# thowell/CALIPSO.jl

Hardware: AMD Instinct MI355X
Metric: Newton steps/sec (n~5k KKT) (higher is better)
Workload: dtype f64; 1 GPU; C3 synthetic dense conic QP: nx=2500 ne=1500 nc=1000 (400 R+ + 200 x SOC3), n=5000 condensed, N=8500 unreduced; ONE system per GPU stepped sequentially (replicas at N > 1); 1 LDL^T factorisation, 6 refinement round(s) per step; refinement_rounds=6

## Files before the change

calipso.jl_amd/__init__.py:

```python
import ctypes as C

import numpy as np

from ._lib import CALLBACK_FN, EVAL_FN, CalipsoHipError, lib

__all__ = ["Solver", "Group", "LDLSolver", "SmallBatch", "Comm", "ordering", "symbolic", "Options", "initialize_b", "solve_b", "CalipsoHipError", "FLAGS", "splitmix_uniform",
           "mfma_f64_peak"]

FLAGS = dict(
    objective=1 << 0, objective_gradient_variables=1 << 1, objective_jacobian_variables_variables=1 << 2,
    equality_constraint=1 << 3, equality_jacobian_variables=1 << 4, equality_dual_jacobian_variables=1 << 5,
    equality_dual_jacobian_variables_variables=1 << 6, cone_constraint=1 << 7, cone_jacobian_variables=1 << 8,
    cone_dual_jacobian_variables=1 << 9, cone_dual_jacobian_variables_variables=1 << 10,
    objective_jacobian_variables_parameters=1 << 11, equality_jacobian_parameters=1 << 12,
    equality_dual_jacobian_variables_parameters=1 << 13, cone_jacobian_parameters=1 << 14,
    cone_dual_jacobian_variables_parameters=1 << 15)
CONE_BARRIER, CONE_BARRIER_GRADIENT, CONE_PRODUCT, CONE_JACOBIAN, CONE_TARGET = 1, 2, 4, 8, 16

STATUS_TEXT = {-1: "inertia correction failure", -2: "cone search failure", -3: "evaluation callback failed",
               -4: "bad argument", -5: "HIP error", -6: "cone layout not supported"}


def _pd(a):
    return a.ctypes.data_as(C.POINTER(C.c_double))
# ... 402 lines not shown
    def newton_steps(self, count, advance=False):
        info = np.zeros(6 * max(int(count), 1))
        status = np.zeros(max(int(count), 1), dtype=np.int32)
        self._check(self._L.calipso_hip_newton_steps(self._h, int(count), int(advance), _pd(info), status.ctypes.data_as(C.POINTER(C.c_int32))), "newton_steps")
        I = info.reshape(-1, 6)
        return [dict(status=int(status[k]), step_size=I[k, 0], step_size_cone_slack_dual=I[k, 1], refinement_rounds=int(I[k, 2]), factorizations=int(I[k, 3]),
                     merit_candidate=I[k, 4], violation_candidate=I[k, 5]) for k in range(int(count))]

    def phase_times(self):
        out = np.zeros(9)
        self._L.calipso_hip_phase_times(self._h, _pd(out))
        return out

    def kernel_times(self):
        out = np.zeros(8)
        self._L.calipso_hip_kernel_times(self._h, _pd(out))
        return out

    def structure_work(self):
        out = np.zeros(8)
        self._check(self._L.calipso_hip_structure_work(self._h, _pd(out)), "structure_work")
        return dict(schur_flops=out[0], packed_doubles=out[1], segment_pairs=int(out[2]), factor_flops=out[3], factor_nnz=out[4], order=int(out[5]), structured=bool(out[6]))

    def padded_nx(self):
        return int(self.kernel_times()[2])

    def device_bytes(self):
        return int(self.kernel_times()[3])

    def analyze_structure(self):
        out = np.zeros(4, dtype=np.int64)
        self._check(self._L.calipso_hip_analyze_structure(self._h, _pi(out)), "analyze_structure")
        return dict(half_bandwidth=int(out[0]), band_blocks=int(out[1]), equality_rows_per_group=int(out[2]), cone_rows_per_group=int(out[3]))

    def clear_structure(self):
        self._check(self._L.calipso_hip_clear_structure(self._h), "clear_structure")

    def set_stage_parallel(self, on=True, batch=1):
        out = np.zeros(4, dtype=np.int64)
        self._check(self._L.calipso_hip_set_stage_parallel(self._h, 1 if on else 0, int(batch), _pi(out)), "set_stage_parallel")
        return dict(levels=int(out[0]), largest_front=int(out[1]), nnz_upper=int(out[2]))

    def set_stage_blocks(self, on=True):
        out = np.zeros(4, dtype=np.int64)
        self._check(self._L.calipso_hip_set_stage_blocks(self._h, 1 if on else 0, _pi(out)), "set_stage_blocks")
        return dict(z_blocks=int(out[0]), hessian_blocks=int(out[1]), segments=int(out[2]), packed_doubles=int(out[3]))
# ... 811 lines not shown
```

calipso.jl_amd/_lib.py:

```python
import ctypes as C
import os

_HERE = os.path.dirname(os.path.abspath(__file__))
LIB_PATH = os.environ.get("CALIPSO_HIP_LIB") or os.path.join(_HERE, "libcalipso_hip.so")
_LIB = None

EVAL_FN = C.CFUNCTYPE(C.c_int32, C.c_void_p, C.c_uint32, C.POINTER(C.c_double), C.POINTER(C.c_double), C.POINTER(C.c_double),
                      C.POINTER(C.c_double))

CALLBACK_FN = C.CFUNCTYPE(None, C.c_void_p, C.c_void_p)
DEVICE_EVAL_FN = C.CFUNCTYPE(C.c_int32, C.c_void_p, C.c_uint32, C.c_void_p, C.c_void_p, C.c_void_p, C.c_void_p, C.c_void_p, C.c_void_p)

_vp, _i32, _i64, _u32, _u64, _dbl = C.c_void_p, C.c_int32, C.c_int64, C.c_uint32, C.c_uint64, C.c_double
_pd, _pi64, _pi32 = C.POINTER(C.c_double), C.POINTER(C.c_int64), C.POINTER(C.c_int32)
SYMBOLS = {
    "calipso_hip_create": (_i32, [_i64, _i64, _i64, _i64, _i64, _pi64, _i64, _pi64, _pi64, _i32, C.POINTER(_vp)]),
    "calipso_hip_create_structured": (_i32, [_i64, _i64, _i64, _i64, _i64, _pi64, _i64, _pi64, _pi64, _i32, _pi64, _pi64, _i64, _pi64, C.POINTER(_vp)]),
    "calipso_hip_destroy": (_i32, [_vp]),
    "calipso_hip_last_error": (C.c_char_p, [_vp]),
    "calipso_hip_version": (C.c_char_p, []),
    "calipso_hip_device_count": (_i32, []),
    "calipso_hip_set_field": (_i32, [_vp, C.c_char_p, _pd, _i64]),
    "calipso_hip_get_field": (_i32, [_vp, C.c_char_p, _pd, _i64]),
    "calipso_hip_set_sparsity": (_i32, [_vp, C.c_char_p, _i64, _pi64, _pi64]),
# ... 20 lines not shown
    "calipso_hip_merit_gradient": (_i32, [_vp]),
    "calipso_hip_constraint_violation": (_i32, [_vp, _i32, _pd]),
    "calipso_hip_merit_directional": (_i32, [_vp, _pd]),
    "calipso_hip_accept": (_i32, [_vp, _dbl]),
    "calipso_hip_initialize": (_i32, [_vp, _pd]),
    "calipso_hip_solve": (_i32, [_vp, EVAL_FN, _vp]),
    "calipso_hip_differentiate": (_i32, [_vp, EVAL_FN, _vp]),
    "calipso_hip_differentiate_info": (_i32, [_vp, _pd]),
    "calipso_hip_differentiate_adjoint": (_i32, [_vp, EVAL_FN, _vp, _i64, _pd, _pd, _pd, C.POINTER(_pd)]),
    "calipso_hip_differentiate_adjoint_info": (_i32, [_vp, _pd]),
    "calipso_hip_differentiate_adjoint_times": (_i32, [_vp, _pd]),
    "calipso_hip_set_device_evaluator": (_i32, [_vp, C.c_void_p, _vp]),
    "calipso_hip_set_device_block_evaluator": (_i32, [_vp, C.c_void_p, _vp]),
    "calipso_hip_device_evaluate": (_i32, [_vp, _i32, _u32]),
    "calipso_hip_set_callbacks": (_i32, [_vp, C.c_void_p, C.c_void_p, _vp]),
    "calipso_hip_stats": (_i32, [_vp, _pi64]),
    "calipso_hip_qp_attach": (_i32, [_vp, _pd, _pd, _pd, _pd, _pd, _pd, _dbl]),
    "calipso_hip_qp_evaluate": (_i32, [_vp, _i32, _u32]),
    "calipso_hip_newton_step": (_i32, [_vp, _i32, _pd]),
    "calipso_hip_newton_steps": (_i32, [_vp, _i32, _i32, _pd, _pi32]),
    "calipso_hip_phase_times": (_i32, [_vp, _pd]),
    "calipso_hip_kernel_times": (_i32, [_vp, _pd]),
    "calipso_hip_structure_work": (_i32, [_vp, _pd]),
    "calipso_hip_analyze_structure": (_i32, [_vp, _pi64]),
    "calipso_hip_clear_structure": (_i32, [_vp]),
    "calipso_hip_set_stage_parallel": (_i32, [_vp, _i32, _i32, _pi64]),
    "calipso_hip_set_stage_blocks": (_i32, [_vp, _i32, _pi64]),
    "calipso_hip_group_create": (_i32, [C.POINTER(_vp), _i32, C.POINTER(_vp)]),
    "calipso_hip_group_destroy": (_i32, [_vp]),
    "calipso_hip_group_newton_step": (_i32, [_vp, _i32, _pd, C.POINTER(_i32)]),
    "calipso_hip_group_solve": (_i32, [_vp, C.POINTER(_i32)]),
    "calipso_hip_group_set_evaluators": (_i32, [_vp, C.POINTER(EVAL_FN), C.POINTER(_vp)]),
    "calipso_hip_group_differentiate_adjoint": (_i32, [_vp, _i64, _pd, _pd, _pd, C.POINTER(_pd), _pi32, _pd]),
    "calipso_hip_group_differentiate": (_i32, [_vp, _pd, _pi32, _i32, _pd]),
    "calipso_hip_ldl_create": (_i32, [_i64, _i32, C.POINTER(_vp)]),
    "calipso_hip_ldl_factorize_csc": (_i32, [_vp, _i64, _pi64, _pi64, _pd, _pi64]),
    "calipso_hip_ldl_inertia": (_i32, [_vp, _pi64]),
    "calipso_hip_ordering": (_i32, [_i64, _pi64, _pi64, _i32, _pi64]),
    "calipso_hip_symbolic": (_i64, [_i64, _pi64, _pi64, _pi64, _pi64, _pi64, _pi64, _pi64, _pi64, _pi64]),
    "calipso_hip_ldl_analyze_csc": (_i32, [_vp, _i64, _pi64, _pi64, _i32, _pi64, _pi64]),
    "calipso_hip_ldl_solve": (_i32, [_vp, _i64, _i64, _pd, _pd]),
    "calipso_hip_sparse_create": (_i32, [_i64, _pi64, _pi64, _i32, _pi64, _i32, C.POINTER(_vp)]),
    "calipso_hip_sparse_destroy": (_i32, [_vp]),
    "calipso_hip_sparse_last_error": (C.c_char_p, [_vp]),
    "calipso_hip_sparse_info": (_i32, [_vp, _pi64]),
    "calipso_hip_sparse_set_batch": (_i32, [_vp, _i64]),
# ... 70 lines not shown
```

calipso.jl_amd/csrc/api.hip:

```cpp
#include <algorithm>
#include <array>
#include <atomic>
#include <cmath>
#include <mutex>
#include <cstdio>
#include <cstdlib>
#include <cstring>

#include "internal.hpp"
#include "device_utils.hpp"
#include "host_logic.hpp"

using namespace calipso;

namespace calipso {
int check(H* s, hipError_t e, const char* what) {
    char buf[512];
    snprintf(buf, sizeof buf, "%s: %s", what, hipGetErrorString(e));
    if (s) s->err = buf;
    return CALIPSO_ERR_HIP;
}
bool lds_attribute(const void* kernel, int bytes) {
    static std::mutex mu;
    static std::map<std::pair<const void*, int>, std::pair<int, int>> done;
// ... 166 lines not shown
        size_t off = 0;
        for (auto& c : carve) { *c.first = s->slab + off; off += (c.second + 31) & ~(size_t)31; }
    }
    s->icount = reinterpret_cast<int*>(icount_d);
    s->krange = reinterpret_cast<int*>(krange_d);
    s->zrow = reinterpret_cast<int*>(zrow_d);
    s->gx = s->Z; s->hx = s->Z + NE; s->g = s->gh; s->hc = s->gh + NE;
    s->Lf = s->S;
    schur_plan(s);
    rc |= dalloc(s, &s->cone.soc_start, (size_t)d.n_soc); rc |= dalloc(s, &s->cone.soc_dim, (size_t)d.n_soc);
    rc |= dalloc(s, &s->cone.soc_woff, (size_t)d.n_soc); rc |= dalloc(s, &s->cone.entry_soc, NC);
    rc |= dalloc(s, &s->cone.wide, (size_t)d.n_wide);
    std::vector<int> zgrp;
    calipso::solve_tail_plan(d, s->h_soc_start, s->h_soc_dim, zgrp);
    if (zgrp.size() >= 2) { rc |= dalloc(s, &s->zgrp, zgrp.size()); s->n_zgrp = (int)zgrp.size() - 1; }
    rc |= dalloc(s, &s->gate, (size_t)4);
    if (rc) return CALIPSO_ERR_HIP;
    CK(hipHostMalloc((void**)&s->hscal, 64 * sizeof(double), hipHostMallocMapped | hipHostMallocCoherent));
    CK(hipHostMalloc((void**)&s->hicount, 64 * sizeof(int), hipHostMallocMapped | hipHostMallocCoherent));
    CK(hipHostMalloc((void**)&s->hseq, 64, hipHostMallocMapped | hipHostMallocCoherent));
    CK(hipHostGetDevicePointer((void**)&s->hscal_dev, s->hscal, 0));
    CK(hipHostGetDevicePointer((void**)&s->hicount_dev, s->hicount, 0));
    CK(hipHostGetDevicePointer((void**)&s->hseq_dev, s->hseq, 0));
    s->hseq[0] = 0;
    CK(hipStreamSynchronize(s->stream));
    {
        std::vector<int> kr(4 * KG);
        for (size_t g = 0; g < KG; ++g) { kr[4 * g] = 0; kr[4 * g + 1] = d.ne; kr[4 * g + 2] = 0; kr[4 * g + 3] = d.nc; }
        CK(hipMemcpy(s->krange, kr.data(), sizeof(int) * kr.size(), hipMemcpyHostToDevice));
    }
    if (s->zgrp) CK(hipMemcpy(s->zgrp, zgrp.data(), sizeof(int) * zgrp.size(), hipMemcpyHostToDevice));
    if (d.n_soc) {
        CK(hipMemcpy(s->cone.soc_start, s->h_soc_start.data(), sizeof(int) * d.n_soc, hipMemcpyHostToDevice));
        CK(hipMemcpy(s->cone.soc_dim, s->h_soc_dim.data(), sizeof(int) * d.n_soc, hipMemcpyHostToDevice));
        CK(hipMemcpy(s->cone.soc_woff, s->h_soc_woff.data(), sizeof(int) * d.n_soc, hipMemcpyHostToDevice));
    }
    if (d.n_wide) {
        std::vector<int> wide;
        for (int j = 0; j < d.n_soc; ++j) if (s->h_soc_dim[j] > 4) wide.push_back(j);
        CK(hipMemcpy(s->cone.wide, wide.data(), sizeof(int) * wide.size(), hipMemcpyHostToDevice));
    }
    std::vector<int> es((size_t)std::max(1, d.nc), -1);
    for (int j = 0; j < d.n_soc; ++j)
        for (int k = 0; k < s->h_soc_dim[j]; ++k) es[s->h_soc_start[j] + k] = j;
    if (d.nc) CK(hipMemcpy(s->cone.entry_soc, es.data(), sizeof(int) * d.nc, hipMemcpyHostToDevice));
    s->hpoint.assign(N, 0.0);
    s->hparams.assign((size_t)d.np, 0.0);
// ... 350 lines not shown
__global__ __launch_bounds__(128) void k_publish_words(const unsigned* __restrict__ src, int words, unsigned* __restrict__ hdst, unsigned long long* __restrict__ hseq,
                                                        unsigned long long seq) {
    if ((int)threadIdx.x < words) hdst[threadIdx.x] = src[threadIdx.x];
    __threadfence_system();
    __syncthreads();
    if (threadIdx.x == 0) __hip_atomic_store(hseq, seq, __ATOMIC_RELEASE, __HIP_MEMORY_SCOPE_SYSTEM);
}
static int wait_published(H* s, unsigned long long seq);
static int publish_and_wait(H* s, const void* dsrc, void* hdst_dev, int words) {
    const unsigned long long seq = ++s->pub_seq;
    hipLaunchKernelGGL(k_publish_words, dim3(1), dim3(128), 0, s->stream, static_cast<const unsigned*>(dsrc), words, static_cast<unsigned*>(hdst_dev), s->hseq_dev, seq);
    return wait_published(s, seq);
}
static int wait_published(H* s, unsigned long long seq) {
    if (launch_errors(s, "a kernel launch of this phase was refused")) return CALIPSO_ERR_HIP;
    hipError_t q = hipSuccess;
    const bool ok = host_wait([&] { return __atomic_load_n(s->hseq, __ATOMIC_ACQUIRE) >= seq; },
                              [&] { q = hipStreamQuery(s->stream); return q == hipErrorNotReady; });
    if (ok) return 0;
    if (q != hipSuccess && q != hipErrorNotReady) return calipso::check(s, q, "publish_and_wait");
    s->err = "scalar read-back did not arrive";
    return CALIPSO_ERR_HIP;
}
static int read_scalars(H* s, int first, int count) { return publish_and_wait(s, s->dscal + first, s->hscal_dev + first, 2 * count); }
static int read_icount(H* s, int first, int count) { return publish_and_wait(s, s->icount + first, s->hicount_dev + first, count); }
static double* point_of(H* s, int which) { return which == 0 ? s->solution : s->candidate; }

static void factor_times(H* s) {
    if (!s->factor_times_pending) return;
    s->factor_times_pending = false;
    if (hipEventSynchronize(s->ev[13]) != hipSuccess) return;
    float ms = 0.f;
    (void)hipEventElapsedTime(&ms, s->ev[10], s->ev[11]); s->phase_ms[1] = ms;
    (void)hipEventElapsedTime(&ms, s->ev[11], s->ev[12]); s->phase_ms[7] = ms;
    (void)hipEventElapsedTime(&ms, s->ev[12], s->ev[13]); s->phase_ms[3] = ms;
    s->kernel_ms[0] = hipEventElapsedTime(&ms, s->ev[12], s->ev[14]) == hipSuccess ? ms : 0.0;
}

static int do_factorize(H* s, int64_t inertia[3], bool rhs_ahead_ok = false) {
    factor_times(s);
    (void)hipEventRecord(s->ev[10], s->stream);
    launch_cone_weights(s);
    s->rhs_ahead = false; s->rhs_joined = false;
    if (rhs_ahead_ok) {
        if (hipStream_t st2 = calipso::ldl_rhs_stream(s)) {
            (void)hipEventRecord(s->ev_side[6], s->stream);
            (void)hipStreamWaitEvent(st2, s->ev_side[6], 0);
            hipStream_t keep = s->stream;
            s->stream = st2;
            launch_residual_symmetric(s, s->residual);
            if (s->d.m) calipso::gemv_t(s, s->d.m, s->d.nx, s->Z, s->d.m, s->t1, s->xbuf, 1.0, 1.0, calipso::SP_Z);
            s->stream = keep;
            s->rhs_ahead = true;
        }
    }
    launch_scale_rows(s);
    calipso::inject_refused_launch(s->stream);
    (void)hipEventRecord(s->ev[11], s->stream);
    launch_schur(s);
    (void)hipEventRecord(s->ev[12], s->stream);
    launch_ldl(s);
    (void)hipEventRecord(s->ev[13], s->stream);
    s->factor_times_pending = true;
    if (s->ldl_failed) { s->ldl_failed = false; SYNC(); return CALIPSO_ERR_HIP; }
    if (s->ldl_pub_seq) {
        if (wait_published(s, s->ldl_pub_seq)) return CALIPSO_ERR_HIP;
    } else {
        if (launch_errors(s, "a kernel launch of the factorisation was refused")) return CALIPSO_ERR_HIP;
        CK(hipMemcpyAsync(s->hicount, s->icount, sizeof(int) * 6, hipMemcpyDeviceToHost, s->stream));
        SYNC();
        factor_times(s);
    }
    s->stats.factorizations += 1;
    s->phase_ms[8] += 1.0;
    const int64_t pos = s->hicount[0] + s->hicount[3], nonpos = s->hicount[1] + s->hicount[4], zero = s->hicount[2] + s->hicount[5];
    inertia[0] = pos; inertia[1] = nonpos; inertia[2] = zero;
    if (zero > 0) { inertia[0] = -1; return CALIPSO_WARN_ZERO_PIVOT; }
    return CALIPSO_OK;
}

static int do_inertia_correction(H* s, int64_t* nfact, bool rhs_ahead_ok = false, const int64_t* first_in = nullptr, int first_rc = 0) {
    const Options& o = s->opt; const Dims& d = s->d;
    int64_t in[3];
    ic_begin(o, s->sc);
// ... 218 lines not shown
    double* pt = point_of(s, which);
    if (s->qp.attached) { launch_qp_evaluate(s, pt, flags); return CALIPSO_OK; }
    if (s->dev_eval || s->dev_block_eval) return device_evaluate(s, pt, flags);
    if (!eval) { s->err = "no evaluation callback and no device evaluator attached"; return CALIPSO_ERR_ARGUMENT; }
    CK(hipMemcpyAsync(s->hpoint.data(), pt, sizeof(double) * s->d.N, hipMemcpyDeviceToHost, s->stream));
    SYNC();
    const double* w = s->hpoint.data();
    const int rc = eval(user, flags, w, w + s->d.oy(), w + s->d.oz(), s->hparams.data());
    if (rc != 0) { s->err = "evaluation callback failed"; return CALIPSO_ERR_CALLBACK; }
    return CALIPSO_OK;
}

static int candidate_merit(H* s, calipso_eval_fn eval, void* user, double* Mh, double* thetah, bool with_dd = false, bool queue_only = false) {
    int rc = evaluate(s, eval, user, 1, CALIPSO_EVAL_OBJECTIVE | CALIPSO_EVAL_EQUALITY | CALIPSO_EVAL_CONE);
    if (rc < 0) return rc;
    launch_cone(s, s->candidate, CALIPSO_CONE_BARRIER | CALIPSO_CONE_BARRIER_GRADIENT);
    launch_merit_and_constraint(s, s->candidate, 4, with_dd ? 3 : 2);
    if (queue_only) return CALIPSO_OK;
    if (wait_published(s, s->pub_seq)) return CALIPSO_ERR_HIP;
    *Mh = s->hscal[4]; *thetah = s->hscal[5];
    return CALIPSO_OK;
}

static int inner_iteration(H* s, calipso_eval_fn eval, void* user, double equality_violation, double cone_product_violation, IterInfo& info,
                           double* eq_viol_out, double* cp_viol_out, bool violations_unread = false) {
    const Options& o = s->opt; Scalars& sc = s->sc; const Dims& d = s->d;
    int rc;
    EV(0);
    rc = evaluate(s, eval, user, 0, CALIPSO_EVAL_OBJECTIVE_GRADIENT | CALIPSO_EVAL_EQUALITY_DUAL_GRADIENT | CALIPSO_EVAL_CONE_DUAL_GRADIENT);
    if (rc < 0) return rc;
    launch_cone(s, s->solution, CALIPSO_CONE_BARRIER | CALIPSO_CONE_BARRIER_GRADIENT);
    launch_merit_and_gradient(s);
    launch_residual(s);
    launch_violations_and_constraint(s, 4, 14);
    uint32_t fl = CALIPSO_EVAL_OBJECTIVE_HESSIAN | CALIPSO_EVAL_EQUALITY_JACOBIAN | CALIPSO_EVAL_CONE_JACOBIAN;
    if (o.constraint_tensor != 0.0) fl |= CALIPSO_EVAL_EQUALITY_DUAL_HESSIAN | CALIPSO_EVAL_CONE_DUAL_HESSIAN;
    const bool spec = spec_step_ok(s);
    const bool ahead = spec && s->spec_ahead_ok;
    const Scalars sc_before = sc;
    int64_t in0[3] = {0, 0, 0};
    int rc0 = 0;
    if (ahead) {
        EV(1);
        rc = evaluate(s, eval, user, 0, fl);
        if (rc < 0) return rc;
        EV(2);
        ic_begin(o, sc);
        rc0 = do_factorize(s, in0, true);
        if (rc0 < 0) return rc0;
    } else if (wait_published(s, s->pub_seq)) return CALIPSO_ERR_HIP;
    auto undo_ahead = [&] {
        if (!ahead) return;
        if (s->rhs_ahead && s->stream2) (void)hipStreamSynchronize(s->stream2);
        s->rhs_ahead = false; s->rhs_joined = false;
        sc.ep = sc_before.ep; sc.ed = sc_before.ed;
        s->stats.factorizations -= 1; s->phase_ms[8] -= 1.0;
        s->spec_ahead_ok = false;
    };
    info.M = s->hscal[4]; info.theta = s->hscal[5];
    const StepNorms norms = step_norms(s->hscal, d.N, d.ne, d.nc);
    if (!ahead) EV(1);
    info.exit_kind = exit_kind(o, sc_before.kappa, norms, equality_violation, cone_product_violation, true);
    if (info.exit_kind != 0) {
        undo_ahead();
        s->spec_ahead_ok = false;
        return CALIPSO_OK;
    }
    s->spec_ahead_ok = norms.optimality > 4.0 * inner_exit_threshold(o, sc_before.kappa) && norms.residual_violation >= o.residual_tolerance;
    if (!ahead) {
        rc = evaluate(s, eval, user, 0, fl);
        if (rc < 0) return rc;
        EV(2);
    }
    s->time_matvec = true;
    int warn = do_search_direction(s, &info.nfact, &info.rounds, ahead ? in0 : nullptr, rc0, spec && d.nc > 0);
    if (warn < 0) return warn;
    double step_size = 1.0, Mh = 0.0, thetah = 0.0;
    bool tail_done = false;
    if (s->refine_pending) {
// ... 418 lines not shown
int32_t calipso_hip_phase_times(H* s, double out[9]) {
    if (!s || !out) return CALIPSO_ERR_ARGUMENT;
    factor_times(s);
    for (int i = 0; i < 9; ++i) out[i] = s->phase_ms[i];
    return CALIPSO_OK;
}

int32_t calipso_hip_kernel_times(H* s, double out[8]) {
    if (!s || !out) return CALIPSO_ERR_ARGUMENT;
    for (int i = 0; i < 8; ++i) out[i] = 0.0;
    factor_times(s);
    out[0] = s->kernel_ms[0];
    out[1] = (double)s->ldl_step_launches;
    out[2] = (double)s->d.NP;
    out[3] = (double)(s->slab_doubles * sizeof(double) + s->scratch_bytes);
    { double lf[8]; calipso::lfac_describe(s, lf); out[6] = s->lfac_last ? 1.0 : (s->lfac_failed ? -1.0 : 0.0); out[7] = lf[5]; }
    if (s->matvec_timed && hipEventSynchronize(s->ev[6]) == hipSuccess) {
        float ms = 0.f;
        if (hipEventElapsedTime(&ms, s->ev[5], s->ev[6]) == hipSuccess) { out[4] = ms; out[5] = 8.0 * ((double)s->d.m * s->d.nx + (double)s->d.nx * s->d.nx); }
    }
    return CALIPSO_OK;
}

int32_t calipso_hip_structure_work(H* s, double out[8]) {
    if (!s || !out) return CALIPSO_ERR_ARGUMENT;
    for (int i = 0; i < 8; ++i) out[i] = 0.0;
    if (s->blocks.on) { out[0] = s->blocks.schur_flops; out[1] = (double)s->blocks.packed; out[2] = (double)s->blocks.npairs; }
    if (s->stage_parallel && s->spS) { double w[3]; calipso::sparse_work(s->spS, w); out[3] = w[0]; out[4] = w[1]; out[5] = w[2]; }
    out[6] = s->compact ? 1.0 : 0.0;
    return CALIPSO_OK;
}

int32_t calipso_hip_splitmix_uniform(uint64_t problem_id, uint64_t stream_id, double lo, double hi, int64_t count, double* out) {
    if (!out && count > 0) return CALIPSO_ERR_ARGUMENT;
    uint64_t state = 0xCA11B50000000000ULL + 4096ULL * problem_id + stream_id;
    for (int64_t i = 0; i < count; ++i) {
        state += 0x9E3779B97F4A7C15ULL;
        uint64_t z = state;
        z = (z ^ (z >> 30)) * 0xBF58476D1CE4E5B9ULL;
        z = (z ^ (z >> 27)) * 0x94D049BB133111EBULL;
        z = z ^ (z >> 31);
        out[i] = lo + (hi - lo) * ((double)(z >> 11) * (1.0 / 9007199254740992.0));
    }
    return CALIPSO_OK;
}

// ... 2 lines not shown
```

calipso.jl_amd/csrc/internal.hpp:

```cpp
#pragma once
#include <hip/hip_runtime.h>
#include <stdint.h>

#include <map>
#include <string>
#include <vector>

#include "../../include/calipso_hip.h"
#include "../../include/calipso_options.hpp"
#include "step_decisions.hpp"
#include "sensitivity_columns.hpp"

namespace calipso {

constexpr int TILE = 128;
constexpr int NB = 64;
constexpr int MAX_SOC_DIM = 1024;
constexpr int TRSV_BLOCK = 2048;
inline int trsv_block(int NP, int limit = TRSV_BLOCK) {
    if (NP <= 512) return NP;
    int tb = 512;
    while (2 * tb <= limit && 2 * tb <= NP) tb *= 2;
    for (;; tb /= 2) { const int rem = NP % tb; if (tb == 512 || (rem & (rem - 1)) == 0) return tb; }
}
// ... 94 lines not shown

}

struct calipso_hip_solver {
    calipso::Dims d;
    calipso::Options opt;
    calipso::Scalars sc;
    calipso::ConeDev cone;
    calipso::QpEval qp;
    calipso::Stats stats;
    struct calipso_hip_group* owner = nullptr;
    const calipso::BatchSc* cur = nullptr;
    double* slab = nullptr; size_t slab_doubles = 0;
    int device = 0;
    hipStream_t stream = nullptr;
    std::string err;
    calipso_callback_fn cb_inner = nullptr, cb_outer = nullptr;
    void* cb_user = nullptr;
    calipso_device_eval_fn dev_eval = nullptr;
    void* dev_eval_user = nullptr;
    calipso_device_block_eval_fn dev_block_eval = nullptr;
    void* dev_block_eval_user = nullptr;
    size_t scratch_bytes = 0;
    bool rhs_ahead = false, rhs_joined = false;
    double *evalL = nullptr, *evalZ = nullptr;
    std::map<std::string, double*> optd;
    std::vector<int> h_soc_start, h_soc_dim, h_soc_woff;
    std::vector<int64_t> h_nonneg, h_soc_ptr, h_soc_idx;
    double* Lxx = nullptr;
    double* Z = nullptr;
    double *gx = nullptr, *hx = nullptr;
    double* Lsym = nullptr;
    bool hessian_dirty = true;
    double *fx = nullptr, *gyx = nullptr, *hzx = nullptr;
    double* gh = nullptr;
    double *g = nullptr, *hc = nullptr;
    double *cone_product = nullptr, *cone_target = nullptr, *barrier_gradient = nullptr;
    double* dscal = nullptr;
    double* hscal = nullptr;
    double* hscal_dev = nullptr;
    unsigned long long* hseq = nullptr;
    unsigned long long* hseq_dev = nullptr;
    unsigned long long pub_seq = 0;
    double *jacobian_parameters = nullptr, *solution_sensitivity = nullptr;
    double *solution = nullptr, *candidate = nullptr, *lambda = nullptr, *parameters = nullptr;
    double *residual = nullptr, *residual_error = nullptr, *step = nullptr, *step_correction = nullptr, *saved_point = nullptr;
// ... 98 lines not shown
void launch_residual(calipso_hip_solver* s);
void launch_violations(calipso_hip_solver* s, int pub_first = 0, int pub_count = 0);
void launch_residual_symmetric(calipso_hip_solver* s, const double* res);
void launch_recover(calipso_hip_solver* s, double* step, const double* res, double* accumulate, int zsx_mode = 0);
void launch_refine_local(calipso_hip_solver* s);
bool launch_solve_tail(calipso_hip_solver* s, int which, bool accumulate, bool with_refine);
bool solve_tail_available(const calipso_hip_solver* s);
void solve_tail_plan(const Dims& d, const std::vector<int>& soc_start, const std::vector<int>& soc_dim, std::vector<int>& grp);
void launch_refine_x(calipso_hip_solver* s, bool publish = false);
void launch_refine_x_fused(calipso_hip_solver* s, bool publish, int nchunk, int it = -1, bool last_queued = false);
void launch_trsv_direct(calipso_hip_solver* s, double* x);
void launch_axpy_points(calipso_hip_solver* s, double step_size, int with_s);
void launch_accept(calipso_hip_solver* s, double step_size);
void launch_axpy_points_batch(calipso_hip_solver* s, const double* step_size, int with_s);
void launch_accept_batch(calipso_hip_solver* s, const double* step_size);
void launch_merit(calipso_hip_solver* s, const double* point);
void launch_merit_gradient(calipso_hip_solver* s);
void launch_merit_and_gradient(calipso_hip_solver* s);
void launch_first_candidate(calipso_hip_solver* s, double a_s, double a_t);
void launch_first_candidate_batch(calipso_hip_solver* s, const double* a_s, const double* a_t);
void launch_first_candidate_from_masks(calipso_hip_solver* s);
void launch_constraint_violation(calipso_hip_solver* s, const double* point, int pub_first = 0, int pub_count = 0);
void launch_merit_and_constraint(calipso_hip_solver* s, const double* point, int pub_first, int pub_count);
void launch_violations_and_constraint(calipso_hip_solver* s, int pub_first = 0, int pub_count = 0);
void launch_dot_merit(calipso_hip_solver* s);
void launch_Hmul(calipso_hip_solver* s, const double* v, double* out);
void launch_residual_error(calipso_hip_solver* s, const double* step);
void launch_add(calipso_hip_solver* s, double* y, const double* x, int len);
void launch_assemble_K(calipso_hip_solver* s);
void gemv_n(calipso_hip_solver* s, int rows, int cols, const double* A, int ld, const double* x, double* y, double alpha, double beta, int kind = SP_DENSE,
            const double* add = nullptr);
void gemv_t(calipso_hip_solver* s, int rows, int cols, const double* A, int ld, const double* x, double* y, double alpha, double beta, int kind = SP_DENSE,
            const double* add = nullptr);
void gemv_t2(calipso_hip_solver* s, int rows, int cols, const double* A, int ld, const double* x1, const double* x2, double* y1, double* y2, int kind = SP_DENSE);
int gemv_refine_pair(calipso_hip_solver* s, const double* x1, const double* x2, double* y1, double* y2, const double* xl, double* yl, bool defer_reduce = false);
void gemv_both(calipso_hip_solver* s, int rows, int cols, const double* A, int ld, const double* x, const double* u, double* yn, double* yt, double beta_t,
               int kind = SP_DENSE);
void launch_cone_weights(calipso_hip_solver* s);
void launch_cone_weights_wide(calipso_hip_solver* s);
void launch_residual_symmetric_wide(calipso_hip_solver* s, const double* res, int p, double* rsym, double* t1, bool regions);
void launch_recover_wide(calipso_hip_solver* s, const double* res, int p, const double* rsym, const double* t2, double* dsym, double* step, double* accumulate, int zsx_mode, bool regions);
void launch_refine_local_wide(calipso_hip_solver* s, int part0);
void launch_scale_rows(calipso_hip_solver* s);
void launch_schur(calipso_hip_solver* s);
void launch_symmetrize(calipso_hip_solver* s);
void schur_plan(calipso_hip_solver* s);
void launch_pad_identity(calipso_hip_solver* s);
// ... 105 lines not shown
```

calipso.jl_amd/csrc/ldl.hip:

```cpp
#include "internal.hpp"
#define LDL_TRACE_OWNER
#include "ldl_device.hpp"
#include "host_logic.hpp"

#include <algorithm>
#include <array>
#include <chrono>
#include <mutex>

namespace calipso {


__global__ __launch_bounds__(DIAG_THREADS) void k_ldl_diag(Batch bt, int NP, int nx, int k0, int tb, double* __restrict__ S, double* __restrict__ Dx,
                                                            double* __restrict__ Tinv, double* __restrict__ Minv, int* __restrict__ icount) {
    __shared__ double smem[DIAG_LDS_DOUBLES];
    inst_shift(bt, S, Dx, Tinv, Minv);
    inst_shift_i(bt, icount);
    const int lane = threadIdx.x & 63, w = threadIdx.x >> 6, R = w >> 2, C = w & 3, fr = lane & 15, fk = lane >> 4;
    v4d acc = (v4d){0.0, 0.0, 0.0, 0.0};
    if (R >= C) {
#pragma unroll
        for (int q = 0; q < 4; ++q) acc[q] = S[(k0 + 16 * R + fr) + (size_t)(k0 + 16 * C + fk + 4 * q) * NP];
    }
    diag_block(smem, acc, NP, nx, k0, tb, S, Dx, Tinv, Minv, icount);
// ... 504 lines not shown
    const int NP = s->d.NP, tb = trsv_block(NP, (int)s->solve_block), tiles = half / 32;
    const Batch bt = batch_of(s).b;
    hipLaunchKernelGGL(k_tinv_merge32, dim3(pairs * tiles * tiles, 1, bt.n), dim3(256), 0, stream, bt, NP, tb, half, phase, pair0, s->Lf, s->Tinv, s->Ttmp + merge_scratch(NP, half));
}
constexpr int WFORM_WGS = 128;
static void ldl_plan_ranges(calipso_hip_solver* s) {
    const int NP = s->d.NP, nblk = NP / NB, tb = trsv_block(NP, (int)s->solve_block);
    s->ldl_ranges.clear();
    s->ldl_feeds.clear();
    const bool wf = wform_on(s);
    std::vector<std::array<int, 3>> feeds;
    for (int b0 = 0; b0 < NP; b0 += tb) {
        const int wblk = std::min(tb, NP - b0), wr = std::min(FEED, wblk);
        for (int c = b0; c < b0 + wblk; c += wr) {
            feeds.push_back({(c + wr) / NB, 0, (int)s->ldl_ranges.size() / 2});
            s->ldl_ranges.push_back(c); s->ldl_ranges.push_back(wr);
        }
        if (wf && b0 + wblk < NP) {
            int step = (b0 + wblk) / NB;
            while (step < nblk - 1) { const int ntr = nblk - 1 - step; if (ntr * (ntr + 1) / 2 + WFORM_WGS <= 248) break; ++step; }
            feeds.push_back({step, 1, b0 / tb});
        }
    }
    std::stable_sort(feeds.begin(), feeds.end(), [](const std::array<int, 3>& a, const std::array<int, 3>& b) { return a[0] < b[0]; });
    for (const auto& f : feeds) { s->ldl_feeds.push_back(f[0]); s->ldl_feeds.push_back(f[1]); s->ldl_feeds.push_back(f[2]); }
}
static void enqueue_feed(calipso_hip_solver* s, hipStream_t stream, int i, bool beside) {
    const int kind = s->ldl_feeds[3 * i + 1], arg = s->ldl_feeds[3 * i + 2];
    if (kind == 0) { enqueue_finish_feed(s, stream, arg); return; }
    if (!beside) { enqueue_wform(s, stream, arg); return; }
    const int NP = s->d.NP, tb = trsv_block(NP, (int)s->solve_block);
    const int k0 = arg * tb, w = std::min(tb, NP - k0), rb = NP - k0 - w;
    const Batch bt = batch_of(s).b;
    const int rows = wform_rows(s, rb);
    hipLaunchKernelGGL(k_wform_product64, dim3(std::min(WFORM_WGS, (rows / 64) * (w / 64)), 1, bt.n), dim3(1024), 0, stream, bt, NP, tb, arg, w, rb, rows, s->Lf, s->Tinv, s->Wfac + wform_offset(NP, tb, arg));
}
static void enqueue_finish_feed(calipso_hip_solver* s, hipStream_t stream, int f) {
    const int NP = s->d.NP, nblk = NP / NB, tb = trsv_block(NP, (int)s->solve_block);
    const Batch bt = batch_of(s).b;
    const unsigned nz = bt.n;
    const int c0 = s->ldl_ranges[2 * f], w = s->ldl_ranges[2 * f + 1];
    const int b0 = c0 / tb * tb, wblk = std::min(tb, NP - b0);
    const int p0 = c0 / NB, np = std::min(w / NB, nblk - 1 - p0);
    if (np > 0) hipLaunchKernelGGL(k_ldl_scale, dim3((NP - p0 * NB - NB) / 64, np, nz), dim3(1024), 0, stream, bt, NP, tb, NP, p0, s->S, s->Lf, s->Dx, s->Tinv);
    for (int half = 64; 2 * half <= w; half *= 2)
        for (int phase = 0; phase < 2; ++phase) enqueue_merge(s, stream, half, phase, c0 / (2 * half), w / (2 * half));
    int rel = c0 - b0;
    bool block_done = w == wblk;
    for (int cur = w; 2 * cur <= wblk; cur *= 2) {
        const int pair = (b0 + (rel & ~(2 * cur - 1))) / (2 * cur);
        if ((rel & (2 * cur - 1)) == 0) { enqueue_merge(s, stream, cur, 0, pair, 1); break; }
        enqueue_merge(s, stream, cur, 1, pair, 1);
// ... 408 lines not shown
```

calipso.jl_amd/csrc/vectors.hip:

```cpp
#include <algorithm>
#include <mutex>

#include "internal.hpp"
#include "device_utils.hpp"

namespace calipso {

constexpr int RT = 1024;

__global__ void k_residual(BatchSc bt, Dims d, const double* __restrict__ w, const double* __restrict__ lam,
                           const double* __restrict__ fx, const double* __restrict__ gyx, const double* __restrict__ hzx,
                           const double* __restrict__ g, const double* __restrict__ hc, const double* __restrict__ prod,
                           const double* __restrict__ targ, double* __restrict__ res) {
    inst_shift(bt.b, w, lam, fx, gyx, hzx, g, hc, prod, targ, res);
    const Scalars sc = bt.scal(blockIdx.z);
    const int i = blockIdx.x * blockDim.x + threadIdx.x;
    if (i >= d.N) return;
    double v;
    if (i < d.orr()) {
        v = fx[i];
        v += gyx[i];
        v += hzx[i];
    } else if (i < d.os()) {
        const int k = i - d.orr();
// ... 557 lines not shown
    const bool pub = pub_count > 0 && !s->cur;
    hipLaunchKernelGGL(k_constraint_violation, dim3(1, 1, B.b.n), dim3(RT), 0, s->stream, B.b, s->d, norm_type(s->opt.constraint_norm), point, s->g,
                       s->hc, s->dscal, pub_first, pub_count, pub ? s->hscal_dev : (double*)nullptr, pub ? s->hseq_dev : (unsigned long long*)nullptr,
                       pub ? ++s->pub_seq : 0ULL);
}

__global__ __launch_bounds__(RT) void k_merit_and_constraint(BatchSc bt, Dims d, int ptype, const double* __restrict__ point, const double* __restrict__ lam,
                                                              const double* __restrict__ g, const double* __restrict__ hc, double* __restrict__ dscal, int pub_first,
                                                              int pub_count, double* __restrict__ hpub, unsigned long long* __restrict__ hseq, unsigned long long seq) {
    __shared__ double sm[RT / 64];
    inst_shift(bt.b, point, lam, g, hc, dscal);
    merit_body(bt.scal(blockIdx.z), d, point, lam, dscal, sm);
    __syncthreads();
    constraint_violation_body(d, ptype, point, g, hc, dscal);
    publish_tail(dscal, pub_first, pub_count, hpub, hseq, seq);
}
void launch_merit_and_constraint(calipso_hip_solver* s, const double* point, int pub_first, int pub_count) {
    const BatchSc B = batch_of(s);
    const bool pub = pub_count > 0 && !s->cur;
    hipLaunchKernelGGL(k_merit_and_constraint, dim3(1, 1, B.b.n), dim3(RT), 0, s->stream, B, s->d, norm_type(s->opt.constraint_norm), point, s->lambda, s->g, s->hc, s->dscal,
                       pub_first, pub_count, pub ? s->hscal_dev : (double*)nullptr, pub ? s->hseq_dev : (unsigned long long*)nullptr, pub ? ++s->pub_seq : 0ULL);
}

void launch_violations_and_constraint(calipso_hip_solver* s, int pub_first, int pub_count) {
    const BatchSc B = batch_of(s);
    const bool pub = pub_count > 0 && !s->cur;
    hipLaunchKernelGGL(k_violations_and_constraint, dim3(1, 1, B.b.n), dim3(RT), 0, s->stream, B.b, s->d, norm_type(s->opt.residual_norm), norm_type(s->opt.constraint_norm),
                       s->residual, s->solution, s->g, s->cone_product, s->hc, s->dscal, pub_first, pub_count, pub ? s->hscal_dev : (double*)nullptr,
                       pub ? s->hseq_dev : (unsigned long long*)nullptr, pub ? ++s->pub_seq : 0ULL);
}

__device__ __forceinline__ void dot_body(int n, const double* __restrict__ a, const double* __restrict__ b, double* __restrict__ out, double* sm) {
    double acc = 0.0;
    for (int i0 = threadIdx.x; i0 < n; i0 += 4 * RT) {
        double av[4], bv[4];
#pragma unroll
        for (int u = 0; u < 4; ++u) { const int i = i0 + u * RT; av[u] = i < n ? a[i] : 0.0; bv[u] = i < n ? b[i] : 0.0; }
#pragma unroll
        for (int u = 0; u < 4; ++u) if (i0 + u * RT < n) acc += av[u] * bv[u];
    }
    const double r = block_sum(acc, sm);
    if (threadIdx.x == 0) *out = r;
}
__global__ __launch_bounds__(RT) void k_dot(Batch bt, int n, const double* __restrict__ a, const double* __restrict__ b, double* __restrict__ out) {
    __shared__ double sm[RT / 64];
    inst_shift(bt, a, b, out);
    dot_body(n, a, b, out, sm);
}
void launch_dot_merit(calipso_hip_solver* s) {
    const BatchSc B = batch_of(s);
    hipLaunchKernelGGL(k_dot, dim3(1, 1, B.b.n), dim3(RT), 0, s->stream, B.b, s->d.n, s->merit_gradient, s->step, s->dscal + 6);
}
// ... 872 lines not shown
```

include/calipso_hip.h:

```cpp
#ifndef CALIPSO_HIP_H
#define CALIPSO_HIP_H

#include <stdint.h>

#ifdef __cplusplus
extern "C" {
#endif

typedef struct calipso_hip_solver calipso_hip_solver;

enum {
    CALIPSO_OK = 0,
    CALIPSO_ERR_INERTIA = -1,
    CALIPSO_ERR_CONE_SEARCH = -2,
    CALIPSO_ERR_CALLBACK = -3,
    CALIPSO_ERR_ARGUMENT = -4,
    CALIPSO_ERR_HIP = -5,
    CALIPSO_ERR_LAYOUT = -6,
    CALIPSO_WARN_ZERO_PIVOT = 1,
    CALIPSO_WARN_REFINEMENT = 2,
    CALIPSO_WARN_LINE_SEARCH = 3
};

enum {
// ... 223 lines not shown
int32_t calipso_hip_smallnewton_initialize_device(calipso_hip_smallnewton*, const double* x0);
int32_t calipso_hip_smallnewton_set_state_device(calipso_hip_smallnewton*, const double* w, const double* lambda, const double* scalars);
int32_t calipso_hip_smallnewton_set_parameters_device(calipso_hip_smallnewton*, const double* theta, int32_t shared);
int32_t calipso_hip_smallnewton_solve_device(calipso_hip_smallnewton*);
int32_t calipso_hip_smallnewton_get_solution_device(calipso_hip_smallnewton*, double* x, double* y, double* z, double* w, int32_t* status);
int32_t calipso_hip_smallnewton_differentiate_adjoint_device(calipso_hip_smallnewton*, int64_t k, const double* cot_w, const double* cot_x, const double* cot_y, const double* cot_z,
                                                             double* adjoint, double* grad_theta, double* const* grad_qp, int32_t reduce_mask, int32_t row_major, int32_t* status);

typedef struct calipso_hip_comm calipso_hip_comm;
int32_t calipso_hip_comm_unique_id(uint8_t id[128]);
int32_t calipso_hip_comm_init(int32_t rank, int32_t nranks, const uint8_t id[128], int32_t device, calipso_hip_comm** out);
int32_t calipso_hip_comm_destroy(calipso_hip_comm*);
int32_t calipso_hip_comm_size(calipso_hip_comm*, int32_t out[2]);
const char* calipso_hip_comm_last_error(calipso_hip_comm*);
int64_t calipso_hip_comm_gather_status(calipso_hip_comm*, const int32_t* rows, int64_t n_rows, int32_t* all_rows, int64_t cap_rows,
                                       int64_t* counts_out);
int32_t calipso_hip_comm_allreduce_sum(calipso_hip_comm*, double* values, int64_t count);

int32_t calipso_hip_mfma_f64_peak(int32_t device, double* tflops);

int32_t calipso_hip_phase_times(calipso_hip_solver*, double out[9]);
int32_t calipso_hip_kernel_times(calipso_hip_solver*, double out[8]);
int32_t calipso_hip_structure_work(calipso_hip_solver*, double out[8]);
int32_t calipso_hip_synchronize(calipso_hip_solver*);
int32_t calipso_hip_streams_concurrent(calipso_hip_solver* a, calipso_hip_solver* b, double out[6]);
int32_t calipso_hip_rebind_stream(calipso_hip_solver*, int32_t priority_class);

int32_t calipso_hip_splitmix_uniform(uint64_t problem_id, uint64_t stream_id, double lo, double hi, int64_t count, double* out);

#ifdef __cplusplus
}
#endif
#endif
```

Measured before the change: 543.4 Newton steps/s.

## Overlap step prologue with LDL factorisation via side-stream feed

```diff
diff --git a/calipso.jl_amd/__init__.py b/calipso.jl_amd/__init__.py
--- a/calipso.jl_amd/__init__.py
+++ b/calipso.jl_amd/__init__.py
@@ -448,6 +448,11 @@
         self._check(self._L.calipso_hip_structure_work(self._h, _pd(out)), "structure_work")
         return dict(schur_flops=out[0], packed_doubles=out[1], segment_pairs=int(out[2]), factor_flops=out[3], factor_nnz=out[4], order=int(out[5]), structured=bool(out[6]))
 
+    def schedule_info(self):
+        out = np.zeros(4)
+        self._check(self._L.calipso_hip_schedule_info(self._h, _pd(out)), "schedule_info")
+        return dict(prologue_ahead_steps=int(out[0]), last_prologue_mode=int(out[1]), ahead_undone=int(out[2]))
+
     def padded_nx(self):
         return int(self.kernel_times()[2])
 
diff --git a/calipso.jl_amd/_lib.py b/calipso.jl_amd/_lib.py
--- a/calipso.jl_amd/_lib.py
+++ b/calipso.jl_amd/_lib.py
@@ -66,6 +66,7 @@
     "calipso_hip_phase_times": (_i32, [_vp, _pd]),
     "calipso_hip_kernel_times": (_i32, [_vp, _pd]),
     "calipso_hip_structure_work": (_i32, [_vp, _pd]),
+    "calipso_hip_schedule_info": (_i32, [_vp, _pd]),
     "calipso_hip_analyze_structure": (_i32, [_vp, _pi64]),
     "calipso_hip_clear_structure": (_i32, [_vp]),
     "calipso_hip_set_stage_parallel": (_i32, [_vp, _i32, _i32, _pi64]),
diff --git a/calipso.jl_amd/csrc/api.hip b/calipso.jl_amd/csrc/api.hip
--- a/calipso.jl_amd/csrc/api.hip
+++ b/calipso.jl_amd/csrc/api.hip
@@ -212,7 +212,7 @@
     CK(hipHostGetDevicePointer((void**)&s->hscal_dev, s->hscal, 0));
     CK(hipHostGetDevicePointer((void**)&s->hicount_dev, s->hicount, 0));
     CK(hipHostGetDevicePointer((void**)&s->hseq_dev, s->hseq, 0));
-    s->hseq[0] = 0;
+    s->hseq[0] = 0; s->hseq[1] = 0;
     CK(hipStreamSynchronize(s->stream));
     {
         std::vector<int> kr(4 * KG);
@@ -609,6 +609,15 @@
     s->err = "scalar read-back did not arrive";
     return CALIPSO_ERR_HIP;
 }
+static int wait_published_side(H* s, unsigned long long seq) {
+    hipError_t q = hipSuccess;
+    const bool ok = host_wait([&] { return __atomic_load_n(s->hseq + 1, __ATOMIC_ACQUIRE) >= seq; },
+                              [&] { q = hipStreamQuery(s->stream2); return q == hipErrorNotReady; });
+    if (ok) return 0;
+    if (q != hipSuccess && q != hipErrorNotReady) return calipso::check(s, q, "wait_published_side");
+    s->err = "scalar read-back of the second stream did not arrive";
+    return CALIPSO_ERR_HIP;
+}
 static int read_scalars(H* s, int first, int count) { return publish_and_wait(s, s->dscal + first, s->hscal_dev + first, 2 * count); }
 static int read_icount(H* s, int first, int count) { return publish_and_wait(s, s->icount + first, s->hicount_dev + first, count); }
 static double* point_of(H* s, int which) { return which == 0 ? s->solution : s->candidate; }
@@ -630,7 +639,9 @@
     launch_cone_weights(s);
     s->rhs_ahead = false; s->rhs_joined = false;
     if (rhs_ahead_ok) {
-        if (hipStream_t st2 = calipso::ldl_rhs_stream(s)) {
+        hipStream_t st2 = calipso::ldl_rhs_stream(s);
+        if (st2 && s->side_work) s->rhs_ahead = true;
+        else if (st2) {
             (void)hipEventRecord(s->ev_side[6], s->stream);
             (void)hipStreamWaitEvent(st2, s->ev_side[6], 0);
             hipStream_t keep = s->stream;
@@ -646,7 +657,9 @@
     (void)hipEventRecord(s->ev[11], s->stream);
     launch_schur(s);
     (void)hipEventRecord(s->ev[12], s->stream);
+    s->side_ran = false;
     launch_ldl(s);
+    if (s->side_work && s->rhs_ahead && !s->side_ran) s->side_work(s);
     (void)hipEventRecord(s->ev[13], s->stream);
     s->factor_times_pending = true;
     if (s->ldl_failed) { s->ldl_failed = false; SYNC(); return CALIPSO_ERR_HIP; }
@@ -911,39 +924,84 @@
     return CALIPSO_OK;
 }
 
+static int step_prologue(H* s, bool side, calipso_eval_fn eval = nullptr, void* user = nullptr) {
+    const int rc = evaluate(s, eval, user, 0, CALIPSO_EVAL_OBJECTIVE_GRADIENT | CALIPSO_EVAL_EQUALITY_DUAL_GRADIENT | CALIPSO_EVAL_CONE_DUAL_GRADIENT);
+    if (rc < 0) return rc;
+    launch_cone(s, s->solution, CALIPSO_CONE_BARRIER | CALIPSO_CONE_BARRIER_GRADIENT);
+    launch_merit_and_gradient(s);
+    launch_residual(s);
+    launch_violations_and_constraint(s, 4, 14, side);
+    return rc;
+}
+static int prologue_ahead_mode(H* s) {
+    static const int env = [] { const char* e = getenv("CALIPSO_HIP_PROLOGUE_AHEAD"); return e ? atoi(e) : 2; }();
+    if (env <= 0 || calipso::ldl_rhs_stream(s) == nullptr) return 0;
+    return env == 1 ? 1 : 2;
+}
+static void queue_side_work(H* s) {
+    s->side_ran = true;
+    if (s->prologue_pending) {
+        s->prologue_pending = false;
+        s->prologue_rc = step_prologue(s, true);
+        if (s->prologue_rc < 0) return;
+    }
+    launch_residual_symmetric(s, s->residual);
+    if (s->d.m) calipso::gemv_t(s, s->d.m, s->d.nx, s->Z, s->d.m, s->t1, s->xbuf, 1.0, 1.0, calipso::SP_Z);
+}
+
 static int inner_iteration(H* s, calipso_eval_fn eval, void* user, double equality_violation, double cone_product_violation, IterInfo& info,
                            double* eq_viol_out, double* cp_viol_out, bool violations_unread = false) {
     const Options& o = s->opt; Scalars& sc = s->sc; const Dims& d = s->d;
     int rc;
     EV(0);
-    rc = evaluate(s, eval, user, 0, CALIPSO_EVAL_OBJECTIVE_GRADIENT | CALIPSO_EVAL_EQUALITY_DUAL_GRADIENT | CALIPSO_EVAL_CONE_DUAL_GRADIENT);
+    const bool spec = spec_step_ok(s);
+    const bool ahead = spec && s->spec_ahead_ok;
+    const int side = ahead ? prologue_ahead_mode(s) : 0;
+    struct SideWork {
+        H* s; ~SideWork() { s->side_work = nullptr; s->prologue_pending = false; }
+    } side_guard{s};
+    s->last_prologue_mode = side;
+    const unsigned long long side_seq = side ? s->pub_seq2 + 1 : 0;
+    if (side == 1) {
+        (void)hipEventRecord(s->ev_side[5], s->stream);
+        (void)hipStreamWaitEvent(s->stream2, s->ev_side[5], 0);
+        hipStream_t keep = s->stream;
+        s->stream = s->stream2;
+        rc = step_prologue(s, true);
+        s->stream = keep;
+    } else if (side == 2) {
+        s->side_work = queue_side_work; s->prologue_pending = true; s->prologue_rc = 0;
+        rc = 0;
+    } else rc = step_prologue(s, false, eval, user);
     if (rc < 0) return rc;
-    launch_cone(s, s->solution, CALIPSO_CONE_BARRIER | CALIPSO_CONE_BARRIER_GRADIENT);
-    launch_merit_and_gradient(s);
-    launch_residual(s);
-    launch_violations_and_constraint(s, 4, 14);
+    if (side) s->prologue_ahead_steps += 1;
     uint32_t fl = CALIPSO_EVAL_OBJECTIVE_HESSIAN | CALIPSO_EVAL_EQUALITY_JACOBIAN | CALIPSO_EVAL_CONE_JACOBIAN;
     if (o.constraint_tensor != 0.0) fl |= CALIPSO_EVAL_EQUALITY_DUAL_HESSIAN | CALIPSO_EVAL_CONE_DUAL_HESSIAN;
-    const bool spec = spec_step_ok(s);
-    const bool ahead = spec && s->spec_ahead_ok;
     const Scalars sc_before = sc;
     int64_t in0[3] = {0, 0, 0};
     int rc0 = 0;
+    auto drain_side = [&] {
+        if ((side || s->rhs_ahead) && s->stream2) (void)hipStreamSynchronize(s->stream2);
+        s->rhs_ahead = false; s->rhs_joined = false;
+    };
     if (ahead) {
         EV(1);
         rc = evaluate(s, eval, user, 0, fl);
-        if (rc < 0) return rc;
+        if (rc < 0) { drain_side(); return rc; }
         EV(2);
         ic_begin(o, sc);
         rc0 = do_factorize(s, in0, true);
-        if (rc0 < 0) return rc0;
+        if (rc0 >= 0 && side && s->prologue_rc < 0) rc0 = s->prologue_rc;
+        if (rc0 < 0) { drain_side(); return rc0; }
+        if (side && wait_published_side(s, side_seq)) { drain_side(); return CALIPSO_ERR_HIP; }
     } else if (wait_published(s, s->pub_seq)) return CALIPSO_ERR_HIP;
     auto undo_ahead = [&] {
         if (!ahead) return;
-        if (s->rhs_ahead && s->stream2) (void)hipStreamSynchronize(s->stream2);
+        if ((side || s->rhs_ahead) && s->stream2) (void)hipStreamSynchronize(s->stream2);
         s->rhs_ahead = false; s->rhs_joined = false;
         sc.ep = sc_before.ep; sc.ed = sc_before.ed;
         s->stats.factorizations -= 1; s->phase_ms[8] -= 1.0;
+        s->ahead_undone += 1;
         s->spec_ahead_ok = false;
     };
     info.M = s->hscal[4]; info.theta = s->hscal[5];
@@ -1408,6 +1466,12 @@
     return CALIPSO_OK;
 }
 
+int32_t calipso_hip_schedule_info(H* s, double out[4]) {
+    if (!s || !out) return CALIPSO_ERR_ARGUMENT;
+    out[0] = (double)s->prologue_ahead_steps; out[1] = (double)s->last_prologue_mode; out[2] = (double)s->ahead_undone; out[3] = 0.0;
+    return CALIPSO_OK;
+}
+
 int32_t calipso_hip_structure_work(H* s, double out[8]) {
     if (!s || !out) return CALIPSO_ERR_ARGUMENT;
     for (int i = 0; i < 8; ++i) out[i] = 0.0;
diff --git a/calipso.jl_amd/csrc/internal.hpp b/calipso.jl_amd/csrc/internal.hpp
--- a/calipso.jl_amd/csrc/internal.hpp
+++ b/calipso.jl_amd/csrc/internal.hpp
@@ -140,6 +140,13 @@
     calipso_device_block_eval_fn dev_block_eval = nullptr;
     void* dev_block_eval_user = nullptr;
     size_t scratch_bytes = 0;
+    int last_prologue_mode = 0;
+    bool prologue_pending = false, side_ran = false;
+    int prologue_rc = 0;
+    void (*side_work)(calipso_hip_solver*) = nullptr;
+    unsigned long long pub_seq2 = 0;
+    long long prologue_ahead_steps = 0;
+    long long ahead_undone = 0;
     bool rhs_ahead = false, rhs_joined = false;
     double *evalL = nullptr, *evalZ = nullptr;
     std::map<std::string, double*> optd;
@@ -284,7 +291,7 @@
 void launch_first_candidate_from_masks(calipso_hip_solver* s);
 void launch_constraint_violation(calipso_hip_solver* s, const double* point, int pub_first = 0, int pub_count = 0);
 void launch_merit_and_constraint(calipso_hip_solver* s, const double* point, int pub_first, int pub_count);
-void launch_violations_and_constraint(calipso_hip_solver* s, int pub_first = 0, int pub_count = 0);
+void launch_violations_and_constraint(calipso_hip_solver* s, int pub_first = 0, int pub_count = 0, bool side = false);
 void launch_dot_merit(calipso_hip_solver* s);
 void launch_Hmul(calipso_hip_solver* s, const double* v, double* out);
 void launch_residual_error(calipso_hip_solver* s, const double* step);
diff --git a/calipso.jl_amd/csrc/ldl.hip b/calipso.jl_amd/csrc/ldl.hip
--- a/calipso.jl_amd/csrc/ldl.hip
+++ b/calipso.jl_amd/csrc/ldl.hip
@@ -550,12 +550,23 @@
             feeds.push_back({step, 1, b0 / tb});
         }
     }
+    if (s->side_work) {
+        const int step = std::max(0, std::min(nblk - 2, 2));
+        feeds.push_back({step, 2, 0});
+    }
     std::stable_sort(feeds.begin(), feeds.end(), [](const std::array<int, 3>& a, const std::array<int, 3>& b) { return a[0] < b[0]; });
     for (const auto& f : feeds) { s->ldl_feeds.push_back(f[0]); s->ldl_feeds.push_back(f[1]); s->ldl_feeds.push_back(f[2]); }
 }
 static void enqueue_feed(calipso_hip_solver* s, hipStream_t stream, int i, bool beside) {
     const int kind = s->ldl_feeds[3 * i + 1], arg = s->ldl_feeds[3 * i + 2];
     if (kind == 0) { enqueue_finish_feed(s, stream, arg); return; }
+    if (kind == 2) {
+        hipStream_t keep = s->stream;
+        s->stream = stream;
+        if (s->side_work) s->side_work(s);
+        s->stream = keep;
+        return;
+    }
     if (!beside) { enqueue_wform(s, stream, arg); return; }
     const int NP = s->d.NP, tb = trsv_block(NP, (int)s->solve_block);
     const int k0 = arg * tb, w = std::min(tb, NP - k0), rb = NP - k0 - w;
diff --git a/calipso.jl_amd/csrc/vectors.hip b/calipso.jl_amd/csrc/vectors.hip
--- a/calipso.jl_amd/csrc/vectors.hip
+++ b/calipso.jl_amd/csrc/vectors.hip
@@ -603,12 +603,13 @@
                        pub_first, pub_count, pub ? s->hscal_dev : (double*)nullptr, pub ? s->hseq_dev : (unsigned long long*)nullptr, pub ? ++s->pub_seq : 0ULL);
 }
 
-void launch_violations_and_constraint(calipso_hip_solver* s, int pub_first, int pub_count) {
+void launch_violations_and_constraint(calipso_hip_solver* s, int pub_first, int pub_count, bool side) {
     const BatchSc B = batch_of(s);
     const bool pub = pub_count > 0 && !s->cur;
+    unsigned long long* const word = !pub ? (unsigned long long*)nullptr : (side ? s->hseq_dev + 1 : s->hseq_dev);
+    const unsigned long long seq = !pub ? 0ULL : (side ? ++s->pub_seq2 : ++s->pub_seq);
     hipLaunchKernelGGL(k_violations_and_constraint, dim3(1, 1, B.b.n), dim3(RT), 0, s->stream, B.b, s->d, norm_type(s->opt.residual_norm), norm_type(s->opt.constraint_norm),
-                       s->residual, s->solution, s->g, s->cone_product, s->hc, s->dscal, pub_first, pub_count, pub ? s->hscal_dev : (double*)nullptr,
-                       pub ? s->hseq_dev : (unsigned long long*)nullptr, pub ? ++s->pub_seq : 0ULL);
+                       s->residual, s->solution, s->g, s->cone_product, s->hc, s->dscal, pub_first, pub_count, pub ? s->hscal_dev : (double*)nullptr, word, seq);
 }
 
 __device__ __forceinline__ void dot_body(int n, const double* __restrict__ a, const double* __restrict__ b, double* __restrict__ out, double* sm) {
diff --git a/include/calipso_hip.h b/include/calipso_hip.h
--- a/include/calipso_hip.h
+++ b/include/calipso_hip.h
@@ -269,6 +269,7 @@
 int32_t calipso_hip_phase_times(calipso_hip_solver*, double out[9]);
 int32_t calipso_hip_kernel_times(calipso_hip_solver*, double out[8]);
 int32_t calipso_hip_structure_work(calipso_hip_solver*, double out[8]);
+int32_t calipso_hip_schedule_info(calipso_hip_solver*, double out[4]);
 int32_t calipso_hip_synchronize(calipso_hip_solver*);
 int32_t calipso_hip_streams_concurrent(calipso_hip_solver* a, calipso_hip_solver* b, double out[6]);
 int32_t calipso_hip_rebind_stream(calipso_hip_solver*, int32_t priority_class);
```

Measured after the change: 559.4 Newton steps/s, median of 6. 2.9% higher.
